# Distributed-Deep-Learning/MiniPs

Hardware: AMD Instinct MI355X
Metric: samples/sec (whole node) Criteo-shaped Wide&Deep BSP at 1/2/4/8 MI355X (higher is better)
Workload: dtype bf16; 1 GPU; global_batch=16384, parallelism=ps-dp1 (bsp; single rank: local shards, no collectives), per_gpu_batch=16384, consistency=bsp, world_size=1, backend=none, lookahead=2

## Files before the change

### csrc/kernels/widedeep.hip

```cpp
#include <cstdlib>
#include <stdexcept>
#include <string>
#include <utility>
#include <vector>

#include "common.h"
#include "kernels.h"

namespace minips_k {

__global__ void wd_assemble_kernel(const float* __restrict__ dense, int n_dense, const bf16_t* __restrict__ rows,
                                   int row_stride, const int64_t* __restrict__ inv, int64_t B, int F, int D,
                                   bf16_t* __restrict__ X, int ldx, float* __restrict__ wide_logit, int ones_col,
                                   float* __restrict__ zero_out) {
  if (zero_out && blockIdx.x == 0 && threadIdx.x == 0) *zero_out = 0.f;
  const int chunks = ldx >> 3;
  const int emb_cols = F * D;
  const int64_t total = B * chunks;
  const int64_t total_r = (total + 63) & ~63ll;
  for (int64_t c = blockIdx.x * (int64_t)blockDim.x + threadIdx.x; c < total_r + 32 * B;
       c += (int64_t)gridDim.x * blockDim.x) {
    if (c >= total_r) {
      const int64_t k = c - total_r, b = k >> 5;
      const int f = (int)(k & 31);
      float w = f < F ? bf2f(rows[inv[b * F + f] * row_stride + D]) : 0.f;
#pragma unroll
      for (int o = 16; o > 0; o >>= 1) w += __shfl_xor(w, o, 64);
      if (f == 0) wide_logit[b] = w;
      continue;
    }
    if (c >= total) continue;
    const int64_t b = c / chunks;
    const int col0 = (int)(c - b * chunks) * 8;
    uint32_t packed[4];
    if (col0 + 8 <= emb_cols && (D & 7) == 0) {
      const int f = col0 / D, d = col0 - f * D;
      const bf16_t* src = rows + inv[b * F + f] * row_stride + d;
      const uint2 lo = *reinterpret_cast<const uint2*>(src);
      const uint2 hi = *reinterpret_cast<const uint2*>(src + 4);
      packed[0] = lo.x;
      packed[1] = lo.y;
      packed[2] = hi.x;
      packed[3] = hi.y;
    } else {
      float v[8];
#pragma unroll
      for (int j = 0; j < 8; ++j) {
        const int col = col0 + j;
        if (col < emb_cols) {
          const int f = col / D, d = col - f * D;
          v[j] = bf2f(rows[inv[b * F + f] * row_stride + d]);
        } else if (col < emb_cols + n_dense) {
          v[j] = dense[b * n_dense + (col - emb_cols)];
        } else {
          v[j] = col == ones_col ? 1.f : 0.f;
        }
      }
#pragma unroll
      for (int j = 0; j < 4; ++j) packed[j] = pack_bf2(v[2 * j], v[2 * j + 1]);
    }
    *reinterpret_cast<uint4*>(X + b * ldx + col0) = make_uint4(packed[0], packed[1], packed[2], packed[3]);
  }
}

void wd_assemble(const float* dense, int n_dense, const bf16_t* rows, int row_stride, const int64_t* inv, int64_t B,
                 int F, int D, bf16_t* X, int ldx, float* wide_logit, int ones_col, hipStream_t s, float* zero_out) {
  if (ldx % 8) throw std::runtime_error("wd_assemble: ldx must be a multiple of 8");
  if (F * D + n_dense > ldx) throw std::runtime_error("wd_assemble: ldx too small");
  if (ones_col >= ldx) throw std::runtime_error("wd_assemble: ones_col out of range");
  if (row_stride % 4) throw std::runtime_error("wd_assemble: row_stride must be a multiple of 4");
  if (B <= 0) return;
  const int block = 256;
  if (F > 32) throw std::runtime_error("wd_assemble: at most 32 features");
  const int64_t items = ((B * (ldx / 8) + 63) & ~63ll) + 32 * B;
  hipLaunchKernelGGL(wd_assemble_kernel, (int)((items + block - 1) / block), block, 0, s, dense, n_dense, rows,
                     row_stride, inv, B, F, D, X, ldx, wide_logit, ones_col, zero_out);
  MINIPS_HIP_CHECK(hipGetLastError());
}

__global__ void wd_assemble_tab_kernel(const float* __restrict__ dense, int n_dense, const float* __restrict__ tab,
                                       int64_t tab_ld, const int64_t* __restrict__ uniq, int64_t base,
                                       const int64_t* __restrict__ inv, int64_t B, int F, int D,
                                       bf16_t* __restrict__ X, int ldx, float* __restrict__ wide_logit, int ones_col,
                                       float* __restrict__ zero_out, const int32_t* __restrict__ rowidx) {
  if (zero_out && blockIdx.x == 0 && threadIdx.x == 0) *zero_out = 0.f;
  const int chunks = ldx >> 3;
  const int emb_cols = F * D;
  const int64_t total = B * chunks;
  const int64_t total_r = (total + 63) & ~63ll;
  auto row_of = [&](int64_t b, int f) {
    const int64_t r = rowidx ? (int64_t)rowidx[b * F + f] : uniq[inv[b * F + f]];
    return tab + (r - base) * tab_ld;
  };
  for (int64_t c = blockIdx.x * (int64_t)blockDim.x + threadIdx.x; c < total_r + 32 * B;
       c += (int64_t)gridDim.x * blockDim.x) {
    if (c >= total_r) {
      const int64_t k = c - total_r, b = k >> 5;
      const int f = (int)(k & 31);
      float w = f < F ? __uint_as_float(pack_bf2(row_of(b, f)[D], 0.f) << 16) : 0.f;
#pragma unroll
      for (int o = 16; o > 0; o >>= 1) w += __shfl_xor(w, o, 64);
      if (f == 0) wide_logit[b] = w;
      continue;
    }
    if (c >= total) continue;
    const int64_t b = c / chunks;
    const int col0 = (int)(c - b * chunks) * 8;
    uint32_t packed[4];
    if (col0 + 8 <= emb_cols && (D & 7) == 0) {
      const int f = col0 / D, d = col0 - f * D;
      const float* src = row_of(b, f) + d;
      const float4 lo = *reinterpret_cast<const float4*>(src);
      const float4 hi = *reinterpret_cast<const float4*>(src + 4);
      packed[0] = pack_bf2(lo.x, lo.y);
      packed[1] = pack_bf2(lo.z, lo.w);
      packed[2] = pack_bf2(hi.x, hi.y);
      packed[3] = pack_bf2(hi.z, hi.w);
    } else {
      float v[8];
#pragma unroll
      for (int j = 0; j < 8; ++j) {
        const int col = col0 + j;
        if (col < emb_cols) {
          const int f = col / D, d = col - f * D;
          v[j] = __uint_as_float(pack_bf2(row_of(b, f)[d], 0.f) << 16);
        } else if (col < emb_cols + n_dense) {
          v[j] = dense[b * n_dense + (col - emb_cols)];
        } else {
          v[j] = col == ones_col ? 1.f : 0.f;
        }
      }
#pragma unroll
      for (int j = 0; j < 4; ++j) packed[j] = pack_bf2(v[2 * j], v[2 * j + 1]);
    }
    *reinterpret_cast<uint4*>(X + b * ldx + col0) = make_uint4(packed[0], packed[1], packed[2], packed[3]);
  }
}

void wd_assemble_tab(const float* dense, int n_dense, const float* tab, int64_t tab_ld, const int64_t* uniq,
                     int64_t base, const int64_t* inv, int64_t B, int F, int D, bf16_t* X, int ldx,
                     float* wide_logit, int ones_col, hipStream_t s, float* zero_out, const int32_t* rowidx) {
  if (ldx % 8) throw std::runtime_error("wd_assemble_tab: ldx must be a multiple of 8");
  if (F * D + n_dense > ldx) throw std::runtime_error("wd_assemble_tab: ldx too small");
  if (ones_col >= ldx) throw std::runtime_error("wd_assemble_tab: ones_col out of range");
  if (tab_ld % 4 || (D & 7) || tab_ld < D + 1) throw std::runtime_error("wd_assemble_tab: 16-byte rows, D % 8 == 0");
  if (F > 32) throw std::runtime_error("wd_assemble_tab: at most 32 features");
  if (B <= 0) return;
  const int block = 256;
  const int64_t items = ((B * (ldx / 8) + 63) & ~63ll) + 32 * B;
  hipLaunchKernelGGL(wd_assemble_tab_kernel, (int)((items + block - 1) / block), block, 0, s, dense, n_dense, tab,
                     tab_ld, uniq, base, inv, B, F, D, X, ldx, wide_logit, ones_col, zero_out, rowidx);
  MINIPS_HIP_CHECK(hipGetLastError());
// ... 519 lines not shown

__device__ __forceinline__ int block_excl_scan256(int v, int* sh, int* total) {
  const int lane = threadIdx.x & 63, w = threadIdx.x >> 6;
  int x = v;
#pragma unroll
  for (int o = 1; o < 64; o <<= 1) {
    const int y = __shfl_up(x, o, 64);
    if (lane >= o) x += y;
  }
  if (lane == 63) sh[w] = x;
  __syncthreads();
  int base = 0;
  for (int i = 0; i < w; ++i) base += sh[i];
  *total = sh[0] + sh[1] + sh[2] + sh[3];
  __syncthreads();
  return base + x - v;
}

__global__ __launch_bounds__(256) void emb_scan_reduce_kernel(const int* __restrict__ counts, int U,
                                                              int* __restrict__ tile_sums) {
  __shared__ int sh[4];
  const int i0 = blockIdx.x * kScanTile + threadIdx.x * 4;
  int v = 0;
#pragma unroll
  for (int q = 0; q < 4; ++q) v += (i0 + q < U) ? counts[i0 + q] : 0;
  int tot;
  block_excl_scan256(v, sh, &tot);
  if (threadIdx.x == 0) tile_sums[blockIdx.x] = tot;
}

__global__ __launch_bounds__(256) void emb_scan_top_kernel(int* __restrict__ tile_sums, int ntiles) {
  __shared__ int sh[4];
  int carry = 0;
  for (int base = 0; base < ntiles; base += 256) {
    const int i = base + threadIdx.x;
    const int v = i < ntiles ? tile_sums[i] : 0;
    int tot;
    const int ex = block_excl_scan256(v, sh, &tot);
    if (i < ntiles) tile_sums[i] = carry + ex;
    carry += tot;
  }
}

__global__ __launch_bounds__(256) void emb_scan_final_kernel(const int* __restrict__ counts, int U,
                                                             const int* __restrict__ tile_prefix,
                                                             int* __restrict__ offsets) {
  __shared__ int sh[4];
  const int i0 = blockIdx.x * kScanTile + threadIdx.x * 4;
  int c[4], v = 0;
#pragma unroll
  for (int q = 0; q < 4; ++q) {
    c[q] = (i0 + q < U) ? counts[i0 + q] : 0;
    v += c[q];
  }
  int tot;
  int run = tile_prefix[blockIdx.x] + block_excl_scan256(v, sh, &tot);
#pragma unroll
  for (int q = 0; q < 4; ++q) {
    if (i0 + q < U) offsets[i0 + q] = run;
    run += c[q];
  }
  if (blockIdx.x == gridDim.x - 1 && threadIdx.x == 255) offsets[U] = tile_prefix[blockIdx.x] + tot;
}

__global__ __launch_bounds__(kEmbTB) void emb_seg_fill_kernel(const int64_t* __restrict__ inv, int64_t B, int F,
                                                              const int* __restrict__ offsets,
                                                              int* __restrict__ cursor, int* __restrict__ members,
                                                              int* __restrict__ memrow) {
  __shared__ TileDedupe T;
  const int t = threadIdx.x, f = blockIdx.y;
  const int64_t b0 = (int64_t)blockIdx.x * kEmbTB;
  const int nb = (int)min((int64_t)kEmbTB, B - b0);
  int r, di, rank;
  tile_dedupe(T, inv, b0, nb, F, f, t, r, di, rank);
  if (t < T.nd) T.base[t] = offsets[T.rowof[t]] + atomicAdd(cursor + T.rowof[t], T.cnt[t]);
  __syncthreads();
  if (t < nb) {
    const int pos = T.base[di] + rank;
    members[pos] = (int)((b0 + t) * F + f);
    memrow[pos] = r;
  }
}

__device__ __forceinline__ float4 ld_grad4(const float* p) { return *reinterpret_cast<const float4*>(p); }
__device__ __forceinline__ float4 ld_grad4(const bf16_t* p) {
  const uint2 u = *reinterpret_cast<const uint2*>(p);
  return make_float4(__uint_as_float(u.x << 16), __uint_as_float(u.x & 0xffff0000u), __uint_as_float(u.y << 16),
                     __uint_as_float(u.y & 0xffff0000u));
}

template <int VW>
__device__ __forceinline__ void ld_gradv(const bf16_t* p, float (&v)[VW]) {
  if constexpr (VW == 8) {
    const uint4 u = *reinterpret_cast<const uint4*>(p);
    const uint32_t w[4] = {u.x, u.y, u.z, u.w};
#pragma unroll
    for (int e = 0; e < 4; ++e) {
      v[2 * e] = __uint_as_float(w[e] << 16);
      v[2 * e + 1] = __uint_as_float(w[e] & 0xffff0000u);
    }
  } else {
    const float4 f = ld_grad4(p);
    v[0] = f.x; v[1] = f.y; v[2] = f.z; v[3] = f.w;
  }
}
template <int VW>
__device__ __forceinline__ void ld_gradv(const float* p, float (&v)[VW]) {
#pragma unroll
  for (int h = 0; h < VW / 4; ++h) {
    const float4 f = *reinterpret_cast<const float4*>(p + 4 * h);
    v[4 * h] = f.x; v[4 * h + 1] = f.y; v[4 * h + 2] = f.z; v[4 * h + 3] = f.w;
  }
}

template <int VW>
__device__ __forceinline__ void st_row_vals(float* p, const float (&v)[VW]) {
#pragma unroll
  for (int h = 0; h < VW / 4; ++h)
    reinterpret_cast<float4*>(p)[h] = make_float4(v[4 * h], v[4 * h + 1], v[4 * h + 2], v[4 * h + 3]);
}
template <int VW>
__device__ __forceinline__ void st_row_vals(bf16_t* p, const float (&v)[VW]) {
#pragma unroll
  for (int h = 0; h < VW / 4; ++h)
    reinterpret_cast<uint2*>(p)[h] = make_uint2(pack_bf2(v[4 * h], v[4 * h + 1]), pack_bf2(v[4 * h + 2], v[4 * h + 3]));
}
__device__ __forceinline__ void st_scalar(float* p, float v) { *p = v; }
__device__ __forceinline__ void st_scalar(bf16_t* p, float v) { *p = f2bf(v); }

template <typename TO, int D, int VW>
__device__ __forceinline__ void seg_store_row(TO* __restrict__ out, int row_stride, int row, const float (&acc)[VW],
                                              float accw, bool wide, int l) {
  TO* o = out + (int64_t)row * row_stride;
  if ((row_stride & 3) == 0) {
    st_row_vals<VW>(o + VW * l, acc);
  } else {
#pragma unroll
    for (int e = 0; e < VW; ++e) st_scalar(o + VW * l + e, acc[e]);
  }
  if (l == 0)
    for (int c = D; c < row_stride; ++c) st_scalar(o + c, (c == D && wide) ? accw : 0.f);
}

constexpr int seg_part_stride(int D) { return D + 4; }

template <int D, int VW>
__device__ __forceinline__ void seg_store_part(float* __restrict__ part, int64_t slot, const float (&acc)[VW],
                                               float accw, int l) {
  float* o = part + slot * seg_part_stride(D);
  st_row_vals<VW>(o + VW * l, acc);
  if (l == 0) o[D] = accw;
}

template <typename TX, typename TO, int D, int G, int BATCH, bool SORTED, int VW>
__global__ __launch_bounds__(256) void emb_seg_det_kernel(const TX* __restrict__ dX, int ldx,
                                                          const float* __restrict__ dwide, int F,
                                                          const int* __restrict__ members,
                                                          const int* __restrict__ memrow, int total,
                                                          TO* __restrict__ out, int row_stride,
                                                          float* __restrict__ part) {
  constexpr int L = D / VW, PER = 64 / L, PW = PER * G;
  const int lane = threadIdx.x & 63, sub = lane / L, l = lane % L;
  const bool wide = dwide != nullptr;
  const int64_t wave = (blockIdx.x * (int64_t)blockDim.x + threadIdx.x) >> 6;
  const int64_t nw = ((int64_t)gridDim.x * blockDim.x) >> 6;
  for (int64_t piece = wave; piece * PW < total; piece += nw) {
    const int wbase = (int)(piece * PW);
    const int a = wbase + sub * G, b = min(total, a + G);
    const bool has = a < b;
    const int prev_row = (has && a > 0) ? memrow[a - 1] : -1;
    const int next_row = (has && b < total) ? memrow[b] : -1;
    const int wave_prev = wbase > 0 ? memrow[wbase - 1] : -1;
    int cur = -1, rf = -1, rl = -1;
    bool first = true, hasF = false, interior = false, hasL = false;
    float acc[VW], fv[VW], lv[VW];
#pragma unroll
    for (int e = 0; e < VW; ++e) acc[e] = fv[e] = lv[e] = 0.f;
    float accw = 0.f, fw = 0.f, lw = 0.f;
    for (int m0 = a; m0 < b; m0 += BATCH) {
      int u[BATCH], bb[BATCH];
      float v[BATCH][VW];
      float vw[BATCH];
#pragma unroll
      for (int q = 0; q < BATCH; ++q) {
        const int m = m0 + q;
        u[q] = m < b ? memrow[m] : -1;
        const TX* src;
        if (SORTED) {
          src = dX + (int64_t)(m < b ? m : a) * D + VW * l;
          bb[q] = (wide && l == 0 && m < b) ? members[m] / F : 0;
        } else {
          const int j = m < b ? members[m] : members[a];
          bb[q] = j / F;
          const int ff = j - bb[q] * F;
          src = dX + (int64_t)bb[q] * ldx + ff * D + VW * l;
        }
        ld_gradv<VW>(src, v[q]);
        vw[q] = (wide && l == 0 && m < b) ? dwide[bb[q]] : 0.f;
      }
#pragma unroll
      for (int q = 0; q < BATCH; ++q) {
        if (u[q] < 0) break;
        if (u[q] != cur) {
          if (cur >= 0) {
            if (first && cur == prev_row) {
#pragma unroll
              for (int e = 0; e < VW; ++e) fv[e] = acc[e];
              fw = accw;
              hasF = true;
              rf = cur;
            } else {
              seg_store_row<TO, D, VW>(out, row_stride, cur, acc, accw, wide, l);
            }
            first = false;
          }
          cur = u[q];
#pragma unroll
          for (int e = 0; e < VW; ++e) acc[e] = 0.f;
          accw = 0.f;
        }
#pragma unroll
        for (int e = 0; e < VW; ++e) acc[e] += v[q][e];
        accw += vw[q];
      }
    }
    if (cur >= 0) {
      if (first && cur == prev_row) {
#pragma unroll
        for (int e = 0; e < VW; ++e) fv[e] = acc[e];
        fw = accw;
        hasF = true;
        rf = cur;
        interior = cur == next_row;
      } else if (cur == next_row) {
#pragma unroll
        for (int e = 0; e < VW; ++e) lv[e] = acc[e];
        lw = accw;
        hasL = true;
        rl = cur;
      } else {
        seg_store_row<TO, D, VW>(out, row_stride, cur, acc, accw, wide, l);
      }
    }
    float cv[VW];
#pragma unroll
    for (int e = 0; e < VW; ++e) cv[e] = 0.f;
    float cw = 0.f;
    int crow = -1;
    const int src = (lane - L) & 63;
#pragma unroll
    for (int s = 0; s < PER; ++s) {
      float iv[VW];
#pragma unroll
      for (int e = 0; e < VW; ++e) iv[e] = __shfl(cv[e], src, 64);
      const float iw = __shfl(cw, src, 64);
      const int irow = __shfl(crow, src, 64);
      if (sub == s) {
        const bool carried = s > 0 && irow >= 0 && irow == rf;
        if (hasF) {
          float tv[VW];
#pragma unroll
          for (int e = 0; e < VW; ++e) tv[e] = carried ? iv[e] + fv[e] : fv[e];
          const float tw = carried ? iw + fw : fw;
          if (interior) {
#pragma unroll
            for (int e = 0; e < VW; ++e) cv[e] = tv[e];
            cw = tw;
            crow = rf;
          } else {
            if (wbase > 0 && rf == wave_prev) seg_store_part<D, VW>(part, 2 * piece, tv, tw, l);
            else seg_store_row<TO, D, VW>(out, row_stride, rf, tv, tw, wide, l);
#pragma unroll
            for (int e = 0; e < VW; ++e) cv[e] = lv[e];
            cw = lw;
            crow = hasL ? rl : -1;
          }
        } else {
#pragma unroll
          for (int e = 0; e < VW; ++e) cv[e] = lv[e];
          cw = lw;
          crow = hasL ? rl : -1;
        }
      }
    }
    if (sub == PER - 1 && crow >= 0) seg_store_part<D, VW>(part, 2 * piece + 1, cv, cw, l);
  }
}

template <typename TO, int D, int VW, int PW>
__global__ __launch_bounds__(256) void emb_seg_fix_kernel(const int* __restrict__ memrow, int total,
                                                          const float* __restrict__ part, TO* __restrict__ out,
                                                          int row_stride, bool wide) {
  constexpr int L = D / VW, PER = 64 / L, SP = seg_part_stride(D);
  const int lane = threadIdx.x & 63, sub = lane / L, l = lane % L;
  const int64_t npieces = ((int64_t)total + PW - 1) / PW;
  const int64_t wave = (blockIdx.x * (int64_t)blockDim.x + threadIdx.x) >> 6;
  const int64_t nw = ((int64_t)gridDim.x * blockDim.x) >> 6;
  for (int64_t p = wave; p < npieces; p += nw) {
    const int bw = (int)(p * PW), ew = (int)min((int64_t)total, (p + 1) * PW);
    const int r = memrow[ew - 1];
    if (!(ew < total && memrow[ew] == r)) continue;
    if (bw > 0 && memrow[bw] == r && memrow[bw - 1] == r) continue;
    float s[VW];
#pragma unroll
    for (int e = 0; e < VW; ++e) s[e] = 0.f;
    float sw = 0.f;
    constexpr int QPG = 4;
    for (int64_t w0 = p;; w0 += PER * QPG) {
      bool end = false;
#pragma unroll
      for (int k = 0; k < QPG; ++k) {
      const int64_t q = w0 + k * PER + sub;
      const bool valid = q < npieces;
      const int64_t qc = valid ? q : p;
      const int mb = memrow[qc * PW];
      const int64_t eq = min((int64_t)total, (qc + 1) * PW);
      const int me = eq < total ? memrow[eq] : -1;
      const float* ph = part + (2 * qc) * SP;
      const float* pt = ph + SP;
      float vh[VW], vt[VW];
      ld_gradv<VW>(ph + VW * l, vh);
      ld_gradv<VW>(pt + VW * l, vt);
      const float wh = ph[D], wt = pt[D];
      const bool in = valid && (q == p || mb == r);
      const bool through = in && me == r;
      const bool tail = q == p || through;
      if (in) {
#pragma unroll
        for (int e = 0; e < VW; ++e) s[e] += tail ? vt[e] : vh[e];
        sw += tail ? wt : wh;
      }
      end = end || !through;
      }
      if (__any(end)) break;
    }
#pragma unroll
    for (int o = L; o < 64; o <<= 1) {
#pragma unroll
      for (int e = 0; e < VW; ++e) s[e] += __shfl_xor(s[e], o, 64);
      sw += __shfl_xor(sw, o, 64);
    }
    if (sub == 0) seg_store_row<TO, D, VW>(out, row_stride, r, s, sw, wide, l);
  }
}

void emb_build_csr(const int64_t* inv, int64_t B, int F, int U, int* ws, int* members, int* memrow, hipStream_t s,
                   int* zeroed_cc, bool counts_ready) {
  if (B <= 0 || U <= 0) return;
  int* counts = zeroed_cc ? zeroed_cc : ws;
  int* cursor = counts + U;
  int* offsets = zeroed_cc ? ws : cursor + U;
  int* tiles = offsets + U + 1;
  const int ntiles = (U + kScanTile - 1) / kScanTile;
  if (!zeroed_cc) MINIPS_HIP_CHECK(hipMemsetAsync(counts, 0, sizeof(int) * 2 * (size_t)U, s));
  dim3 grid((unsigned)((B + kEmbTB - 1) / kEmbTB), (unsigned)F);
  if (!(counts_ready && zeroed_cc)) hipLaunchKernelGGL(emb_seg_count_kernel, grid, dim3(kEmbTB), 0, s, inv, B,
                                                       F, counts);
  hipLaunchKernelGGL(emb_scan_reduce_kernel, ntiles, 256, 0, s, counts, U, tiles);
  hipLaunchKernelGGL(emb_scan_top_kernel, 1, 256, 0, s, tiles, ntiles);
  hipLaunchKernelGGL(emb_scan_final_kernel, ntiles, 256, 0, s, counts, U, tiles, offsets);
  hipLaunchKernelGGL(emb_seg_fill_kernel, grid, dim3(kEmbTB), 0, s, inv, B, F, offsets, cursor, members, memrow);
  MINIPS_HIP_CHECK(hipGetLastError());
}

constexpr int kSegG = 16, kSegBatch = 8, kSegVW = 4;

constexpr int seg_per_piece(int D) { return (64 / (D / kSegVW)) * kSegG; }

int64_t emb_seg_part_floats(int64_t total, int D) {
  const int64_t pw = seg_per_piece(D);
  return 2 * ((total + pw - 1) / pw) * seg_part_stride(D);
}

template <typename TX, typename TO>
static void emb_seg_det(const TX* dX, int ldx, const float* dwide, int64_t B, int F, int D, const int* members,
                        const int* memrow, TO* out, int row_stride, float* part, hipStream_t s, bool sorted_rows) {
  const int total = (int)(B * F);
  const int64_t pw = seg_per_piece(D);
  const int64_t pieces = (total + pw - 1) / pw;
  const int blocks = (int)std::max<int64_t>(1, std::min<int64_t>((pieces + 3) / 4, 65535));
  const int fix_blocks = (int)std::max<int64_t>(1, std::min<int64_t>((pieces + 3) / 4, 4096));
#define MINIPS_SEG_DET(DD)                                                                                         \
  if (sorted_rows)                                                                                                \
    hipLaunchKernelGGL((emb_seg_det_kernel<TX, TO, DD, kSegG, kSegBatch, true, kSegVW>), blocks, 256, 0, s, dX,    \
                       ldx, dwide, F, members, memrow, total, out, row_stride, part);                             \
  else                                                                                                            \
    hipLaunchKernelGGL((emb_seg_det_kernel<TX, TO, DD, kSegG, kSegBatch, false, kSegVW>), blocks, 256, 0, s, dX,   \
                       ldx, dwide, F, members, memrow, total, out, row_stride, part);                             \
  if (pieces > 1)                                                                                                 \
    hipLaunchKernelGGL((emb_seg_fix_kernel<TO, DD, kSegVW, seg_per_piece(DD)>), fix_blocks, 256, 0, s, memrow,     \
                       total, part, out, row_stride, dwide != nullptr);
  switch (D) {
    case 16:
      MINIPS_SEG_DET(16)
      break;
    case 32:
      MINIPS_SEG_DET(32)
      break;
    case 64:
      MINIPS_SEG_DET(64)
      break;
    default:
      throw std::runtime_error("emb_backward_seg: D must be 16, 32 or 64");
  }
#undef MINIPS_SEG_DET
  MINIPS_HIP_CHECK(hipGetLastError());
}

void emb_backward_csr(const void* dX, bool bf16, int ldx, const float* dwide, int64_t B, int F, int D,
                      const int* members, const int* memrow, void* out, bool out_bf16, int row_stride, float* part,
                      hipStream_t s, bool sorted_rows) {
  if (B <= 0) return;
  if (row_stride < D + (dwide ? 1 : 0)) throw std::runtime_error("emb_backward_csr: row_stride too small");
  if (bf16 && out_bf16)
    emb_seg_det(static_cast<const bf16_t*>(dX), ldx, dwide, B, F, D, members, memrow, static_cast<bf16_t*>(out),
                row_stride, part, s, sorted_rows);
  else if (bf16)
    emb_seg_det(static_cast<const bf16_t*>(dX), ldx, dwide, B, F, D, members, memrow, static_cast<float*>(out),
                row_stride, part, s, sorted_rows);
  else if (out_bf16)
    emb_seg_det(static_cast<const float*>(dX), ldx, dwide, B, F, D, members, memrow, static_cast<bf16_t*>(out),
                row_stride, part, s, sorted_rows);
  else
    emb_seg_det(static_cast<const float*>(dX), ldx, dwide, B, F, D, members, memrow, static_cast<float*>(out),
                row_stride, part, s, sorted_rows);
}

__global__ void emb_csr_positions_kernel(const int* __restrict__ members, int64_t n, int* __restrict__ pos) {
  for (int64_t m = blockIdx.x * (int64_t)blockDim.x + threadIdx.x; m < n; m += (int64_t)gridDim.x * blockDim.x)
    pos[members[m]] = (int)m;
}

void emb_csr_positions(const int* members, int64_t n, int* pos, hipStream_t s) {
  if (n <= 0) return;
  hipLaunchKernelGGL(emb_csr_positions_kernel, grid_for(n, 256, 4096), 256, 0, s, members, n, pos);
  MINIPS_HIP_CHECK(hipGetLastError());
}

void emb_backward_segment(const void* dX, bool bf16, int ldx, const float* dwide, const int64_t* inv, int64_t B, int F,
                          int D, void* out, bool out_bf16, int row_stride, int U, int* ws, float* part, hipStream_t s) {
  if (B <= 0 || U <= 0) return;
  int* members = ws + 3 * U + 1 + (U / 1024 + 1);
  int* memrow = members + B * F;
  emb_build_csr(inv, B, F, U, ws, members, memrow, s);
  emb_backward_csr(dX, bf16, ldx, dwide, B, F, D, members, memrow, out, out_bf16, row_stride, part, s, false);
}

}
```

### minips_amd/ops/__init__.py

```python
from __future__ import annotations

import math

import torch

from .._native import evalk, ftrlk, kernels, optk, wdftrlk

EPI_STORE_F32 = 0
EPI_ATOMIC_F32 = 1
EPI_BIAS_RELU_BF16 = 2
EPI_BIAS_BF16 = 3
EPI_STORE_BF16 = 4
EPI_RELU_MASK_BF16 = 5
EPI_BIAS_GELU_BF16 = 6
EPI_BIAS_GELU_AUX_BF16 = 7
EPI_GELU_GRAD_BF16 = 8
EPI_PERM_ROWS_BF16 = 9
EPI_BIAS_GELU_DAUX_BF16 = 13
EPI_MUL_AUX_BF16 = 14
_L2E = 1.4426950408889634


def _gelu_grad(u):
    k, c = 0.7978845608, 0.044715
# ... 475 lines not shown
        out = torch.empty(B, rows.shape[1], dtype=torch.float32, device=rows.device)
    if _gpu(rows):
        kernels().embedding_bag_fwd(rows, idx, offsets, bool(mean), out)
        return out
    mode = "mean" if mean else "sum"
    out.copy_(torch.nn.functional.embedding_bag(idx, rows, offsets[:-1], mode=mode, include_last_offset=False))
    return out


def embedding_bag_bwd(grad_out, idx, offsets, grad_rows, mean=False):
    if _gpu(grad_out):
        kernels().embedding_bag_bwd(grad_out, idx, offsets, bool(mean), grad_rows)
        return grad_rows
    lens = (offsets[1:] - offsets[:-1])
    bag = torch.repeat_interleave(torch.arange(lens.numel(), device=idx.device), lens)
    g = grad_out[bag]
    if mean:
        g = g / lens[bag].clamp_min(1).unsqueeze(1).to(g.dtype)
    grad_rows.index_add_(0, idx, g)
    return grad_rows


def wd_assemble(dense, rows, inv, F, D, X, wide_logit, ones_col=-1, zero=None):
    if _gpu(X):
        kernels().wd_assemble(dense, rows, inv, int(F), int(D), X, wide_logit, int(ones_col), zero)
        return X, wide_logit
    if zero is not None:
        zero.zero_()
    B = X.shape[0]
    r = rows[inv].view(B, F, rows.shape[1]).float()
    X.zero_()
    X[:, : F * D] = r[:, :, :D].reshape(B, F * D).to(torch.bfloat16)
    X[:, F * D: F * D + dense.shape[1]] = dense.to(torch.bfloat16)
    if ones_col >= 0:
        X[:, ones_col] = 1.0
    wide_logit.copy_(r[:, :, D].sum(1))
    return X, wide_logit


def wd_assemble_tab(dense, table, index, base, inv, F, D, X, wide_logit, ones_col=-1, zero=None, rowidx=None):
    if _gpu(X):
        kernels().wd_assemble_tab(dense, table, index, int(base), inv, int(F), int(D), X, wide_logit, int(ones_col),
                                  zero, rowidx)
        return X, wide_logit
    U = int(inv.max()) + 1 if inv.numel() else 0
    rows = table[index[:U] - base].to(torch.bfloat16)
    return wd_assemble(dense, rows, inv, F, D, X, wide_logit, ones_col, zero)


def wd_head(H, w, b0, wide_logit, labels, dH, dw, db, dwide, loss_sum, dH_colsum=None, grad_scale=1.0,
            defer_fold=False):
    if _gpu(H):
        kernels().wd_head(H, w, b0, wide_logit, labels, dH, dw, db, dwide, loss_sum, dH_colsum, float(grad_scale),
                          bool(defer_fold))
        return
    h = H.float()
    z = h @ w.float() + b0.float() + wide_logit
    y = (labels > 0.5).float()
    p = torch.sigmoid(z)
    dz = (p - y) * grad_scale
    dwide.copy_(dz)
    db += dz.sum()
    loss_sum += (torch.clamp_min(z, 0) - z * y + torch.log1p(torch.exp(-z.abs()))).sum()
    g = torch.where(h > 0, dz.unsqueeze(1) * w.float().unsqueeze(0), torch.zeros_like(h)).to(torch.bfloat16)
    dH.copy_(g)
    dw += (dz.unsqueeze(1) * h).sum(0)
    if dH_colsum is not None:
        dH_colsum += g.float().sum(0)


def wd_head_fold(B, Hd, dw, db, loss_sum, dH_colsum=None):
    if _gpu(dw):
        (kernels() if _REC is None else _REC.lst).wd_head_fold(int(B), int(Hd), dw, db, loss_sum, dH_colsum)


EVAL_LOSS_SCALE = float(1 << 24)


def _eval_bins(acc) -> int:
    NB = (acc.numel() - 2) // 2
    if acc.dtype != torch.int64 or acc.numel() != 2 * NB + 2 or not 32 <= NB <= 8192 or NB & (NB - 1):
        raise RuntimeError(f"acc must be int64 [2*NB + 2] with NB a power of two in [32, 8192], got "
                           f"{acc.dtype} [{acc.numel()}]")
    return NB


def binary_hist(logits, labels, acc):
    NB = _eval_bins(acc)
    if _gpu(logits):
        evalk().binary_hist(logits, labels, acc)
        return
    z = logits.reshape(-1).to(torch.float32)
    y = labels.reshape(-1).to(torch.float32) > 0.5
    ok = ~torch.isnan(z)
    acc[2 * NB + 1] += int((~ok).sum())
    z, y = z[ok], y[ok]
    zc = torch.clamp(z, -16.0, 16.0)
    bins = torch.clamp_max(torch.floor((zc + 16.0) * float(NB // 32)).to(torch.int64), NB - 1)
    acc[:NB] += torch.bincount(bins[~y], minlength=NB)
    acc[NB:2 * NB] += torch.bincount(bins[y], minlength=NB)
    zl = torch.clamp(z, -64.0, 64.0)
    l = torch.clamp_min(zl, 0) - zl * y.to(torch.float32) + torch.log1p(torch.exp(-zl.abs()))
    acc[2 * NB] += torch.round(l * EVAL_LOSS_SCALE).to(torch.int64).sum()


def eval_head(H, w, b0, wide, labels, acc, logits_out=None):
    if _gpu(H):
        evalk().eval_head_hist(H, w, b0, wide, labels, acc, logits_out)
        return
    z = H.float() @ w.float() + b0.float()
    if wide is not None:
        z = z + wide
    if logits_out is not None:
        logits_out.copy_(z)
    binary_hist(z, labels, acc)


def emb_csr_positions(members):
    if _gpu(members):
        return kernels().emb_csr_positions(members)
    pos = torch.empty_like(members)
    pos[members.long()] = torch.arange(members.numel(), dtype=members.dtype)
    return pos


def emb_build_csr(inv, F, U, zeroed=None, counts_ready=False):
    if _gpu(inv):
        return tuple(kernels().emb_build_csr(inv, int(F), int(max(U, 1)), zeroed, bool(counts_ready)))
    order = torch.sort(inv, stable=True).indices
    return order.to(torch.int32), inv[order].to(torch.int32)


def wd_emb_backward(dX, dwide, inv, F, D, grad_rows, x_off=0, csr=None, sorted_rows=False):
    if _gpu(dX):
        members, memrow = (csr[0], csr[1]) if csr is not None else (None, None)
        kernels().wd_emb_backward(dX, dwide, inv, int(F), int(D), grad_rows, int(x_off), members, memrow,
                                  bool(sorted_rows))
        return grad_rows
    if sorted_rows:
        un = torch.empty_like(dX)
        un[csr[0].long()] = dX
        dX, x_off = un.reshape(-1, F * D), 0
    B = dX.shape[0]
    g = dX[:, x_off: x_off + F * D].float().reshape(B * F, D)
    acc = grad_rows if grad_rows.dtype == torch.float32 else grad_rows.float()
    acc[:, :D].index_add_(0, inv, g)
    if dwide is not None:
        acc[:, D].index_add_(0, inv, dwide.repeat_interleave(F))
    if acc is not grad_rows:
        grad_rows.copy_(acc)
    return grad_rows


def _slab_args(slabs):
    return [(s, int(n), int(p), int(o)) for s, n, p, o in slabs]


def _fold_slabs(g, slabs, group4=True):
    if not slabs:
        return g
    x = g.clone()
    for s, n, p, o in slabs:
        P, r = s[: n * p].view(n, p), x[o: o + p]
        z = 0
        while group4 and z + 3 < n:
            r += (P[z] + P[z + 1]) + (P[z + 2] + P[z + 3])
            z += 4
        while z < n:
            r += P[z]
            z += 1
    return x


def adam_apply(w, m, v, g, lr, beta1=0.9, beta2=0.999, eps=1e-8, weight_decay=0.0, step=1, grad_scale=1.0,
               w_bf16=None, step_dev=None, zero_g=False, slabs=()):
    if _gpu(w):
        kernels().adam_apply(w, m, v, g, float(lr), float(beta1), float(beta2), float(eps), float(weight_decay),
                             int(step), float(grad_scale), w_bf16, step_dev, bool(zero_g), _slab_args(slabs))
        return
    g_in, g = g, _fold_slabs(g, slabs)
    if step_dev is not None:
        step = int(step_dev.reshape(-1)[0])
    gg = g * grad_scale
    m.mul_(beta1).add_((1 - beta1) * gg)
    v.mul_(beta2).add_((1 - beta2) * gg * gg)
    bc1, bc2 = 1 - beta1 ** step, 1 - beta2 ** step
    w.sub_(lr * ((m / bc1) / ((v / bc2).sqrt() + eps) + weight_decay * w))
    if w_bf16 is not None:
        w_bf16.copy_(w.to(torch.bfloat16))
    if zero_g:
        g_in.zero_()


def grad_sumsq(g, part, L=None, slabs=()):
    L = part.numel() if L is None else int(L)
    if _gpu(g):
        optk().grad_sumsq(g, _slab_args(slabs), part, L)
        return part
    if not 1 <= L <= 1024 or part.numel() < L or part.dtype != torch.float64:
        raise RuntimeError(f"grad_sumsq: part must be float64 with 1 <= L <= 1024 entries, got {part.dtype} "
                           f"[{part.numel()}], L {L}")
    part[:L] = 0
    part[0] = _fold_slabs(g, slabs).double().square().sum()
    return part


def clip_scale(total: float, max_norm: float):
    if not math.isfinite(total):
        return math.sqrt(total) if total > 0 else float("nan"), 0.0, True
    norm = math.sqrt(total)
    sd = max_norm / (norm + 1e-6)
    return norm, (float(torch.tensor(sd, dtype=torch.float32)) if sd < 1.0 else 1.0), False


def adam_clip_apply(w, m, v, g, lr, part, max_norm, stats, beta1=0.9, beta2=0.999, eps=1e-8, weight_decay=0.0,
                    step=1, np=None, w_bf16=None, step_dev=None, zero_g=False, slabs=(), write_stats=True):
    np = part.numel() if np is None else int(np)
    if _gpu(w):
        optk().adam_clip_apply(w, m, v, g, _slab_args(slabs), float(lr), float(beta1), float(beta2), float(eps),
                               float(weight_decay), int(step), step_dev, w_bf16, bool(zero_g), part, np,
                               float(max_norm), stats, bool(write_stats))
        return
    if not 1 <= np <= 4096 or part.numel() < np:
        raise RuntimeError(f"adam_clip_apply: np {np} outside [1, 4096] or beyond part [{part.numel()}]")
    norm, scale, skip = clip_scale(float(part[:np].sum()), float(max_norm))
    if write_stats:
        stats[0], stats[1] = norm, scale
        stats[3 if skip else 2] += 1.0 if skip or scale < 1.0 else 0.0
    if not skip:
        adam_apply(w, m, v, _fold_slabs(g, slabs), lr, beta1, beta2, eps, weight_decay, step, scale, w_bf16,
                   step_dev=step_dev)
    if zero_g:
        g.zero_()


def slab_pack(g, out, slabs=()):
    if _gpu(g):
        kernels().slab_pack(g, out, _slab_args(slabs))
        return out
    out.copy_(_fold_slabs(g, slabs, group4=False))
    g.zero_()
    return out


def sgd_apply(w, g, lr, grad_scale=1.0, w_bf16=None):
    if _gpu(w):
        kernels().sgd_apply(w, g, float(lr), float(grad_scale), w_bf16)
        return
    w.sub_(lr * grad_scale * g)
    if w_bf16 is not None:
        w_bf16.copy_(w.to(torch.bfloat16))


def adagrad_apply(w, acc, g, lr, eps=1e-10, grad_scale=1.0, w_bf16=None):
    if _gpu(w):
        kernels().adagrad_apply(w, acc, g, float(lr), float(eps), float(grad_scale), w_bf16)
        return
    gg = g * grad_scale
    acc.add_(gg * gg)
    w.sub_(lr * gg / (acc.sqrt() + eps))
    if w_bf16 is not None:
        w_bf16.copy_(w.to(torch.bfloat16))


def cast_f32_bf16(x, y):
    if _gpu(x):
        kernels().cast_f32_bf16(x, y)
        return y
    y.copy_(x.to(torch.bfloat16))
    return y


def lr_sparse_step(rowptr, cols, vals, labels, w, alpha, delta=None, correct=None):
    if _gpu(w):
        kernels().lr_sparse_step(rowptr, cols, vals, labels, w, float(alpha), delta, correct)
        return
    B = labels.numel()
    lens = rowptr[1:] - rowptr[:-1]
    row = torch.repeat_interleave(torch.arange(B, device=w.device), lens)
    dot = torch.zeros(B, dtype=w.dtype, device=w.device).index_add_(0, row, w[cols] * vals)
    p = torch.sigmoid(dot)
    y = labels.clamp_min(0)
    err = alpha * (y - p)
    if delta is not None:
        delta.index_add_(0, cols, err[row] * vals)
    if correct is not None:
        correct += ((p > 0.5) == (y > 0.5)).float().sum()


def kmeans_assign_csr(rowptr, cols, vals, C, assign=None, dist=None):
    n = rowptr.numel() - 1
    if assign is None:
        assign = torch.empty(n, dtype=torch.int32, device=C.device)
    if _gpu(C):
        cnorm = torch.empty(C.shape[0], dtype=torch.float32, device=C.device)
        kernels().kmeans_assign_csr(rowptr, cols, vals, C, cnorm, assign, dist)
        return assign
    lens = rowptr[1:] - rowptr[:-1]
    row = torch.repeat_interleave(torch.arange(n, device=C.device), lens)
    ok = cols < C.shape[1]
    xn = torch.zeros(n, dtype=torch.float32).index_add_(0, row, vals * vals)
    dots = torch.zeros(n, C.shape[0], dtype=torch.float32)
    dots.index_add_(0, row[ok], vals[ok, None] * C[:, cols[ok]].t())
    d2 = xn[:, None] - 2 * dots + (C * C).sum(1)[None]
    best, idx = d2.min(1)
    assign.copy_(idx.to(torch.int32))
# ... 301 lines not shown
```

Measured before the change: 49.03 million samples/s.

## Restructure segmented embedding backward with prefetched keys, lane-shared indices and magic division

The deterministic segmented-sum embedding backward kernel now loads each group's member/row keys cooperatively, spreading them across lanes and broadcasting them with shuffles. It prefetches the next piece's keys while the current piece accumulates, replaces integer division by F with a magic-multiply that is self-checked on the host, and uses 32-bit offsets when the data fits. The fix kernel runs one wave per block and double-buffers its partial loads. Launch uses 64-thread blocks with a capped grid that can be overridden by an environment variable. The aim is to cut memory latency and integer-op overhead in the gradient scatter, at the cost of more register pressure and more code complexity.

```diff
diff --git a/csrc/kernels/widedeep.hip b/csrc/kernels/widedeep.hip
--- a/csrc/kernels/widedeep.hip
+++ b/csrc/kernels/widedeep.hip
@@ -1,3 +1,4 @@
+#include <atomic>
 #include <cstdlib>
 #include <stdexcept>
 #include <string>
@@ -823,80 +824,156 @@
   if (l == 0) o[D] = accw;
 }
 
-template <typename TX, typename TO, int D, int G, int BATCH, bool SORTED, int VW>
+struct SegDiv {
+  uint32_t mul;
+  int shift;
+};
+static SegDiv seg_div_magic(int F) {
+  int s = 0;
+  while ((1ll << s) < F) ++s;
+  return SegDiv{(uint32_t)((((uint64_t)1 << (31 + s)) + (uint64_t)F - 1) / (uint64_t)F), s};
+}
+__host__ __device__ __forceinline__ int seg_div(int j, SegDiv d) {
+#if defined(__HIP_DEVICE_COMPILE__)
+  return (int)(__umulhi((uint32_t)j << 1, d.mul) >> d.shift);
+#else
+  return (int)((uint32_t)((((uint64_t)(uint32_t)j << 1) * d.mul) >> 32) >> d.shift);
+#endif
+}
+
+struct SegRawBf { uint2 u; };
+struct SegRawF { float4 f; };
+__device__ __forceinline__ SegRawBf seg_ld_raw(const bf16_t* p) { return SegRawBf{*reinterpret_cast<const uint2*>(p)}; }
+__device__ __forceinline__ SegRawF seg_ld_raw(const float* p) { return SegRawF{*reinterpret_cast<const float4*>(p)}; }
+__device__ __forceinline__ SegRawBf seg_pad_raw(const SegRawBf& r, bool valid) {
+  return SegRawBf{make_uint2(valid ? r.u.x : 0x80008000u, valid ? r.u.y : 0x80008000u)};
+}
+__device__ __forceinline__ SegRawF seg_pad_raw(const SegRawF& r, bool valid) {
+  return SegRawF{make_float4(valid ? r.f.x : -0.f, valid ? r.f.y : -0.f, valid ? r.f.z : -0.f, valid ? r.f.w : -0.f)};
+}
+__device__ __forceinline__ void seg_add_raw(float (&acc)[4], const SegRawBf& r) {
+  acc[0] += __uint_as_float(r.u.x << 16);
+  acc[1] += __uint_as_float(r.u.x & 0xffff0000u);
+  acc[2] += __uint_as_float(r.u.y << 16);
+  acc[3] += __uint_as_float(r.u.y & 0xffff0000u);
+}
+__device__ __forceinline__ void seg_add_raw(float (&acc)[4], const SegRawF& r) {
+  acc[0] += r.f.x; acc[1] += r.f.y; acc[2] += r.f.z; acc[3] += r.f.w;
+}
+
+template <typename TO, int D, int VW>
+__device__ __forceinline__ void seg_flush_row(TO* __restrict__ out, int row_stride, int row, const float (&acc)[VW],
+                                              float accw, bool wide, int l) {
+  if (row_stride == D + 4) {
+    TO* o = out + (int64_t)row * (D + 4);
+    st_row_vals<VW>(o + VW * l, acc);
+    if (l == 0) {
+      const float t[4] = {wide ? accw : 0.f, 0.f, 0.f, 0.f};
+      st_row_vals<4>(o + D, t);
+    }
+  } else {
+    seg_store_row<TO, D, VW>(out, row_stride, row, acc, accw, wide, l);
+  }
+}
+
+template <typename TX, typename TO, int D, int G, bool SORTED, int VW, typename OffT>
 __global__ __launch_bounds__(256) void emb_seg_det_kernel(const TX* __restrict__ dX, int ldx,
-                                                          const float* __restrict__ dwide, int F,
-                                                          const int* __restrict__ members,
-                                                          const int* __restrict__ memrow, int total,
-                                                          TO* __restrict__ out, int row_stride,
-                                                          float* __restrict__ part) {
-  constexpr int L = D / VW, PER = 64 / L, PW = PER * G;
-  const int lane = threadIdx.x & 63, sub = lane / L, l = lane % L;
+                                                         const float* __restrict__ dwide, int F, SegDiv fdiv,
+                                                         const int* __restrict__ members,
+                                                         const int* __restrict__ memrow, int total,
+                                                         TO* __restrict__ out, int row_stride,
+                                                         float* __restrict__ part) {
+  static_assert(VW == 4 && G % (D / VW) == 0, "a lane holds 4 values and a whole share of its group's entries");
+  constexpr int L = D / VW, PER = 64 / L, PW = PER * G, E = G / L;
+  const int lane = threadIdx.x & 63, sub = lane / L, l = lane % L, gbase = lane - l;
+  const int wv = __builtin_amdgcn_readfirstlane(threadIdx.x >> 6), wpb = blockDim.x >> 6;
   const bool wide = dwide != nullptr;
-  const int64_t wave = (blockIdx.x * (int64_t)blockDim.x + threadIdx.x) >> 6;
-  const int64_t nw = ((int64_t)gridDim.x * blockDim.x) >> 6;
-  for (int64_t piece = wave; piece * PW < total; piece += nw) {
+  struct Keys {
+    int mu[E], mj[E], wp, wn;
+  };
+  auto load_keys = [&](int64_t pc, Keys& k) {
+    const int wb = (int)(pc * PW);
+    const int ka = (int)min((int64_t)wb + sub * G, (int64_t)total);
+#pragma unroll
+    for (int e = 0; e < E; ++e) {
+      const int idx = ka + min(l * E + e, total - 1 - ka);
+      k.mu[e] = memrow[idx];
+      k.mj[e] = (!SORTED || wide) ? members[idx] : 0;
+    }
+    k.wp = memrow[max(wb - 1, 0)];
+    k.wn = memrow[(int)min((int64_t)wb + PW, (int64_t)total - 1)];
+  };
+  const int64_t npieces = ((int64_t)total + PW - 1) / PW, stride = (int64_t)gridDim.x * wpb;
+  int64_t piece = (int64_t)blockIdx.x * wpb + wv;
+  if (piece >= npieces) return;
+  const float* wsrc = wide ? dwide : reinterpret_cast<const float*>(memrow);
+  const uint32_t wmask = wide ? 0xffffffffu : 0u;
+  Keys kc;
+  load_keys(piece, kc);
+  for (;;) {
     const int wbase = (int)(piece * PW);
-    const int a = wbase + sub * G, b = min(total, a + G);
-    const bool has = a < b;
-    const int prev_row = (has && a > 0) ? memrow[a - 1] : -1;
-    const int next_row = (has && b < total) ? memrow[b] : -1;
-    const int wave_prev = wbase > 0 ? memrow[wbase - 1] : -1;
-    int cur = -1, rf = -1, rl = -1;
-    bool first = true, hasF = false, interior = false, hasL = false;
+    const int a = (int)min((int64_t)wbase + sub * G, (int64_t)total);
+    const int cnt = min(G, total - a);
+    int mu[E], mj[E];
+#pragma unroll
+    for (int e = 0; e < E; ++e) mu[e] = kc.mu[e], mj[e] = kc.mj[e];
+    const int wp = kc.wp, wn = kc.wn;
+    const int wave_prev = wbase > 0 ? wp : -1;
+    const int wave_next = (int64_t)wbase + PW < total ? wn : -1;
+    OffT mo[E];
+    float mw[E];
+#pragma unroll
+    for (int e = 0; e < E; ++e) {
+      const int bb = seg_div(mj[e], fdiv);
+      if (SORTED) mo[e] = (OffT)(a + min(l * E + e, total - 1 - a)) * D;
+      else mo[e] = (OffT)bb * ldx + (mj[e] - bb * F) * D;
+      mw[e] = __uint_as_float(__float_as_uint(wsrc[bb & wmask]) & wmask);
+    }
+    int u[G];
+    decltype(seg_ld_raw(dX)) raw[G];
+#pragma unroll
+    for (int q = 0; q < G; ++q) {
+      u[q] = __shfl(mu[q % E], gbase + q / E, 64);
+      const OffT off = __shfl(mo[q % E], gbase + q / E, 64);
+      raw[q] = seg_ld_raw(dX + off + VW * l);
+    }
+    const int64_t nxt = piece + stride;
+    if (nxt < npieces) load_keys(nxt, kc);
+    const int up = __shfl(mu[E - 1], (gbase - 1) & 63, 64), un = __shfl(mu[0], (gbase + L) & 63, 64);
+    const int prev_row = a > 0 ? (sub > 0 ? up : wave_prev) : -1;
+    const int next_row = (int64_t)a + G < total ? (sub < PER - 1 ? un : wave_next) : -1;
+    float vw[G];
+#pragma unroll
+    for (int q = 0; q < G; ++q) vw[q] = __shfl(mw[q % E], gbase + q / E, 64);
+    int rf = -1, rl = -1;
+    bool pendF = cnt > 0 && u[0] == prev_row, hasF = false, interior = false, hasL = false;
     float acc[VW], fv[VW], lv[VW];
 #pragma unroll
     for (int e = 0; e < VW; ++e) acc[e] = fv[e] = lv[e] = 0.f;
     float accw = 0.f, fw = 0.f, lw = 0.f;
-    for (int m0 = a; m0 < b; m0 += BATCH) {
-      int u[BATCH], bb[BATCH];
-      float v[BATCH][VW];
-      float vw[BATCH];
-#pragma unroll
-      for (int q = 0; q < BATCH; ++q) {
-        const int m = m0 + q;
-        u[q] = m < b ? memrow[m] : -1;
-        const TX* src;
-        if (SORTED) {
-          src = dX + (int64_t)(m < b ? m : a) * D + VW * l;
-          bb[q] = (wide && l == 0 && m < b) ? members[m] / F : 0;
+#pragma unroll
+    for (int q = 0; q < G; ++q) {
+      if (q > 0 && u[q] != u[q - 1]) {
+        if (pendF) {
+#pragma unroll
+          for (int e = 0; e < VW; ++e) fv[e] = acc[e];
+          fw = accw;
+          hasF = true;
+          rf = u[q - 1];
+          pendF = false;
         } else {
-          const int j = m < b ? members[m] : members[a];
-          bb[q] = j / F;
-          const int ff = j - bb[q] * F;
-          src = dX + (int64_t)bb[q] * ldx + ff * D + VW * l;
+          seg_flush_row<TO, D, VW>(out, row_stride, u[q - 1], acc, accw, wide, l);
         }
-        ld_gradv<VW>(src, v[q]);
-        vw[q] = (wide && l == 0 && m < b) ? dwide[bb[q]] : 0.f;
+#pragma unroll
+        for (int e = 0; e < VW; ++e) acc[e] = 0.f;
+        accw = 0.f;
       }
-#pragma unroll
-      for (int q = 0; q < BATCH; ++q) {
-        if (u[q] < 0) break;
-        if (u[q] != cur) {
-          if (cur >= 0) {
-            if (first && cur == prev_row) {
-#pragma unroll
-              for (int e = 0; e < VW; ++e) fv[e] = acc[e];
-              fw = accw;
-              hasF = true;
-              rf = cur;
-            } else {
-              seg_store_row<TO, D, VW>(out, row_stride, cur, acc, accw, wide, l);
-            }
-            first = false;
-          }
-          cur = u[q];
-#pragma unroll
-          for (int e = 0; e < VW; ++e) acc[e] = 0.f;
-          accw = 0.f;
-        }
-#pragma unroll
-        for (int e = 0; e < VW; ++e) acc[e] += v[q][e];
-        accw += vw[q];
-      }
-    }
-    if (cur >= 0) {
-      if (first && cur == prev_row) {
+      seg_add_raw(acc, seg_pad_raw(raw[q], q < cnt));
+      accw += q < cnt ? vw[q] : -0.f;
+    }
+    if (cnt > 0) {
+      const int cur = u[G - 1];
+      if (pendF) {
 #pragma unroll
         for (int e = 0; e < VW; ++e) fv[e] = acc[e];
         fw = accw;
@@ -910,7 +987,7 @@
         hasL = true;
         rl = cur;
       } else {
-        seg_store_row<TO, D, VW>(out, row_stride, cur, acc, accw, wide, l);
+        seg_flush_row<TO, D, VW>(out, row_stride, cur, acc, accw, wide, l);
       }
     }
     float cv[VW];
@@ -940,7 +1017,7 @@
             crow = rf;
           } else {
             if (wbase > 0 && rf == wave_prev) seg_store_part<D, VW>(part, 2 * piece, tv, tw, l);
-            else seg_store_row<TO, D, VW>(out, row_stride, rf, tv, tw, wide, l);
+            else seg_flush_row<TO, D, VW>(out, row_stride, rf, tv, tw, wide, l);
 #pragma unroll
             for (int e = 0; e < VW; ++e) cv[e] = lv[e];
             cw = lw;
@@ -955,55 +1032,75 @@
       }
     }
     if (sub == PER - 1 && crow >= 0) seg_store_part<D, VW>(part, 2 * piece + 1, cv, cw, l);
-  }
-}
+    if (nxt >= npieces) break;
+    piece = nxt;
+  }
+}
+
+template <int D, int VW, int PW, int QPG>
+struct SegFixWindow {
+  int mb[QPG], me[QPG];
+  float vh[QPG][VW], vt[QPG][VW], wh[QPG], wt[QPG];
+  __device__ __forceinline__ void load(const int* __restrict__ memrow, int total, const float* __restrict__ part,
+                                       int64_t npieces, int64_t p, int64_t w0, int sub, int l) {
+    constexpr int PER = 64 / (D / VW), SP = seg_part_stride(D);
+#pragma unroll
+    for (int k = 0; k < QPG; ++k) {
+      const int64_t q = w0 + k * PER + sub;
+      const int64_t qc = q < npieces ? q : p;
+      mb[k] = memrow[qc * PW];
+      const int64_t eq = min((int64_t)total, (qc + 1) * PW);
+      const int mk = memrow[min(eq, (int64_t)total - 1)];
+      me[k] = eq < total ? mk : -1;
+      const float* ph = part + (2 * qc) * SP;
+      const float* pt = ph + SP;
+      ld_gradv<VW>(ph + VW * l, vh[k]);
+      ld_gradv<VW>(pt + VW * l, vt[k]);
+      wh[k] = ph[D];
+      wt[k] = pt[D];
+    }
+  }
+};
 
 template <typename TO, int D, int VW, int PW>
-__global__ __launch_bounds__(256) void emb_seg_fix_kernel(const int* __restrict__ memrow, int total,
-                                                          const float* __restrict__ part, TO* __restrict__ out,
-                                                          int row_stride, bool wide) {
-  constexpr int L = D / VW, PER = 64 / L, SP = seg_part_stride(D);
-  const int lane = threadIdx.x & 63, sub = lane / L, l = lane % L;
+__global__ __launch_bounds__(64) void emb_seg_fix_kernel(const int* __restrict__ memrow, int total,
+                                                         const float* __restrict__ part, TO* __restrict__ out,
+                                                         int row_stride, bool wide) {
+  constexpr int L = D / VW, PER = 64 / L;
+  constexpr int QPG = 4;
+  const int lane = threadIdx.x, sub = lane / L, l = lane % L;
   const int64_t npieces = ((int64_t)total + PW - 1) / PW;
-  const int64_t wave = (blockIdx.x * (int64_t)blockDim.x + threadIdx.x) >> 6;
-  const int64_t nw = ((int64_t)gridDim.x * blockDim.x) >> 6;
-  for (int64_t p = wave; p < npieces; p += nw) {
+  for (int64_t p = blockIdx.x; p < npieces; p += gridDim.x) {
     const int bw = (int)(p * PW), ew = (int)min((int64_t)total, (p + 1) * PW);
     const int r = memrow[ew - 1];
-    if (!(ew < total && memrow[ew] == r)) continue;
-    if (bw > 0 && memrow[bw] == r && memrow[bw - 1] == r) continue;
+    const int rnl = memrow[min(ew, total - 1)], rbl = memrow[max(bw - 1, 0)];
+    const int rn = ew < total ? rnl : -1;
+    const int rb = memrow[bw], rbp = bw > 0 ? rbl : -1;
+    SegFixWindow<D, VW, PW, QPG> w;
+    w.load(memrow, total, part, npieces, p, p, sub, l);
+    const bool active = (rn == r) & !((bw > 0) & (rb == r) & (rbp == r));
     float s[VW];
 #pragma unroll
     for (int e = 0; e < VW; ++e) s[e] = 0.f;
     float sw = 0.f;
-    constexpr int QPG = 4;
-    for (int64_t w0 = p;; w0 += PER * QPG) {
+    for (int64_t w0 = p;;) {
       bool end = false;
 #pragma unroll
       for (int k = 0; k < QPG; ++k) {
-      const int64_t q = w0 + k * PER + sub;
-      const bool valid = q < npieces;
-      const int64_t qc = valid ? q : p;
-      const int mb = memrow[qc * PW];
-      const int64_t eq = min((int64_t)total, (qc + 1) * PW);
-      const int me = eq < total ? memrow[eq] : -1;
-      const float* ph = part + (2 * qc) * SP;
-      const float* pt = ph + SP;
-      float vh[VW], vt[VW];
-      ld_gradv<VW>(ph + VW * l, vh);
-      ld_gradv<VW>(pt + VW * l, vt);
-      const float wh = ph[D], wt = pt[D];
-      const bool in = valid && (q == p || mb == r);
-      const bool through = in && me == r;
-      const bool tail = q == p || through;
-      if (in) {
-#pragma unroll
-        for (int e = 0; e < VW; ++e) s[e] += tail ? vt[e] : vh[e];
-        sw += tail ? wt : wh;
+        const int64_t q = w0 + k * PER + sub;
+        const bool in = q < npieces && (q == p || w.mb[k] == r);
+        const bool through = in && w.me[k] == r;
+        const bool tail = q == p || through;
+        if (in) {
+#pragma unroll
+          for (int e = 0; e < VW; ++e) s[e] += tail ? w.vt[k][e] : w.vh[k][e];
+          sw += tail ? w.wt[k] : w.wh[k];
+        }
+        end = end || !through;
       }
-      end = end || !through;
-      }
-      if (__any(end)) break;
+      if (__any(end) || !active) break;
+      w0 += PER * QPG;
+      w.load(memrow, total, part, npieces, p, w0, sub, l);
     }
 #pragma unroll
     for (int o = L; o < 64; o <<= 1) {
@@ -1011,9 +1108,10 @@
       for (int e = 0; e < VW; ++e) s[e] += __shfl_xor(s[e], o, 64);
       sw += __shfl_xor(sw, o, 64);
     }
-    if (sub == 0) seg_store_row<TO, D, VW>(out, row_stride, r, s, sw, wide, l);
-  }
-}
+    if (sub == 0 && active) seg_flush_row<TO, D, VW>(out, row_stride, r, s, sw, wide, l);
+  }
+}
+
 
 void emb_build_csr(const int64_t* inv, int64_t B, int F, int U, int* ws, int* members, int* memrow, hipStream_t s,
                    int* zeroed_cc, bool counts_ready) {
@@ -1034,13 +1132,25 @@
   MINIPS_HIP_CHECK(hipGetLastError());
 }
 
-constexpr int kSegG = 16, kSegBatch = 8, kSegVW = 4;
+constexpr int kSegG = 16, kSegVW = 4;
 
 constexpr int seg_per_piece(int D) { return (64 / (D / kSegVW)) * kSegG; }
 
 int64_t emb_seg_part_floats(int64_t total, int D) {
   const int64_t pw = seg_per_piece(D);
   return 2 * ((total + pw - 1) / pw) * seg_part_stride(D);
+}
+
+static void seg_div_selfcheck(int F, SegDiv d) {
+  static std::atomic<bool> checked[65];
+  if (F <= 64 && checked[F].load(std::memory_order_relaxed)) return;
+  const int64_t lim = (int64_t)1 << 31;
+  for (int64_t base : {(int64_t)0, (int64_t)1 << 20, lim - 1 - 2 * (int64_t)F}) {
+    const int64_t m0 = base / F * F;
+    for (int64_t j = std::max<int64_t>(0, m0 - 2); j <= m0 + 2 * F + 1 && j < lim; ++j)
+      if (seg_div((int)j, d) != (int)(j / F)) throw std::runtime_error("emb_backward_seg: inexact lookup-id division");
+  }
+  if (F <= 64) checked[F].store(true, std::memory_order_relaxed);
 }
 
 template <typename TX, typename TO>
@@ -1049,18 +1159,29 @@
   const int total = (int)(B * F);
   const int64_t pw = seg_per_piece(D);
   const int64_t pieces = (total + pw - 1) / pw;
-  const int blocks = (int)std::max<int64_t>(1, std::min<int64_t>((pieces + 3) / 4, 65535));
-  const int fix_blocks = (int)std::max<int64_t>(1, std::min<int64_t>((pieces + 3) / 4, 4096));
+  const int blocks = (int)std::max<int64_t>(1, std::min<int64_t>(pieces, 1 << 20));
+  constexpr int tpb = 64;
+  static const int gcap = getenv("MINIPS_SEG_GRID") ? atoi(getenv("MINIPS_SEG_GRID")) : 832;
+  int dblocks = (int)((pieces + tpb / 64 - 1) / (tpb / 64));
+  if (gcap > 0) dblocks = std::min(dblocks, gcap);
+  dblocks = std::max(1, std::min(dblocks, 1 << 20));
+  const SegDiv fdiv = seg_div_magic(F);
+  seg_div_selfcheck(F, fdiv);
+  const bool idx32 = (sorted_rows ? (int64_t)total * D : B * (int64_t)ldx) * (int64_t)sizeof(TX) < ((int64_t)1 << 31);
+#define MINIPS_SEG_DET_K(DD, SORTED, OFFT)                                                                         \
+  hipLaunchKernelGGL((emb_seg_det_kernel<TX, TO, DD, kSegG, SORTED, kSegVW, OFFT>), dblocks, tpb, 0, s, dX, ldx,    \
+                     dwide, F, fdiv, members, memrow, total, out, row_stride, part)
 #define MINIPS_SEG_DET(DD)                                                                                         \
-  if (sorted_rows)                                                                                                \
-    hipLaunchKernelGGL((emb_seg_det_kernel<TX, TO, DD, kSegG, kSegBatch, true, kSegVW>), blocks, 256, 0, s, dX,    \
-                       ldx, dwide, F, members, memrow, total, out, row_stride, part);                             \
-  else                                                                                                            \
-    hipLaunchKernelGGL((emb_seg_det_kernel<TX, TO, DD, kSegG, kSegBatch, false, kSegVW>), blocks, 256, 0, s, dX,   \
-                       ldx, dwide, F, members, memrow, total, out, row_stride, part);                             \
+  if (sorted_rows) {                                                                                              \
+    if (idx32) MINIPS_SEG_DET_K(DD, true, int);                                                                    \
+    else MINIPS_SEG_DET_K(DD, true, int64_t);                                                                      \
+  } else {                                                                                                        \
+    if (idx32) MINIPS_SEG_DET_K(DD, false, int);                                                                   \
+    else MINIPS_SEG_DET_K(DD, false, int64_t);                                                                     \
+  }                                                                                                               \
   if (pieces > 1)                                                                                                 \
-    hipLaunchKernelGGL((emb_seg_fix_kernel<TO, DD, kSegVW, seg_per_piece(DD)>), fix_blocks, 256, 0, s, memrow,     \
-                       total, part, out, row_stride, dwide != nullptr);
+    hipLaunchKernelGGL((emb_seg_fix_kernel<TO, DD, kSegVW, seg_per_piece(DD)>), blocks, 64, 0, s, memrow, total,   \
+                       part, out, row_stride, dwide != nullptr);
   switch (D) {
     case 16:
       MINIPS_SEG_DET(16)
@@ -1074,6 +1195,7 @@
     default:
       throw std::runtime_error("emb_backward_seg: D must be 16, 32 or 64");
   }
+#undef MINIPS_SEG_DET_K
 #undef MINIPS_SEG_DET
   MINIPS_HIP_CHECK(hipGetLastError());
 }
diff --git a/minips_amd/ops/__init__.py b/minips_amd/ops/__init__.py
--- a/minips_amd/ops/__init__.py
+++ b/minips_amd/ops/__init__.py
@@ -651,6 +651,127 @@
     return grad_rows
 
 
+_SEG_G = 16
+
+
+def _seg_per_piece(D):
+    return (64 // (D // 4)) * _SEG_G
+
+
+def _seg_div_magic(F):
+    s = 0
+    while (1 << s) < F:
+        s += 1
+    return ((1 << (31 + s)) + F - 1) // F, s
+
+
+def _seg_div(j, F):
+    mul, s = _seg_div_magic(F)
+    return (((2 * j) & 0xFFFFFFFF) * mul >> 32) >> s
+
+
+def _emb_seg_order_ref(dX, dwide, csr, F, D, grad_rows, x_off=0, sorted_rows=False):
+    import numpy as np
+
+    members, memrow = csr[0].numpy().astype(np.int64), csr[1].numpy().astype(np.int64)
+    total, G = len(members), _SEG_G
+    PER, PW = 64 // (D // 4), _seg_per_piece(D)
+    if sorted_rows:
+        X = dX.float().numpy().reshape(total, D)
+    else:
+        B = dX.shape[0]
+        X = dX[:, x_off: x_off + F * D].float().numpy().reshape(B * F, D)[members]
+    V = np.zeros((total, D + 1), np.float32)
+    V[:, :D] = X
+    wide = dwide is not None
+    if wide:
+        V[:, D] = dwide.float().numpy()[members // F]
+    W = grad_rows.shape[1]
+    res = grad_rows.float().numpy().copy()
+    zero = np.zeros(D + 1, np.float32)
+
+    def store(row, v):
+        res[row, :D] = v[:D]
+        if W > D:
+            res[row, D] = v[D] if wide else 0.0
+            res[row, D + 1:] = 0.0
+
+    npieces = (total + PW - 1) // PW
+    head, tail = np.zeros((npieces, D + 1), np.float32), np.zeros((npieces, D + 1), np.float32)
+    for p in range(npieces):
+        wbase = p * PW
+        wave_prev = memrow[wbase - 1] if wbase > 0 else -1
+        cv, crow = zero, -1
+        for s in range(PER):
+            a, b = wbase + s * G, min(total, wbase + (s + 1) * G)
+            fv = lv = zero
+            rf = rl = -1
+            hasF = interior = hasL = False
+            if a < b:
+                prev_row = memrow[a - 1] if a > 0 else -1
+                next_row = memrow[b] if b < total else -1
+                pendF = memrow[a] == prev_row
+                acc = zero.copy()
+                for m in range(a, b):
+                    if m > a and memrow[m] != memrow[m - 1]:
+                        if pendF:
+                            fv, rf, hasF, pendF = acc, memrow[m - 1], True, False
+                        else:
+                            store(memrow[m - 1], acc)
+                        acc = zero.copy()
+                    acc = acc + V[m]
+                cur = memrow[b - 1]
+                if pendF:
+                    fv, rf, hasF, interior = acc, cur, True, cur == next_row
+                elif cur == next_row:
+                    lv, rl, hasL = acc, cur, True
+                else:
+                    store(cur, acc)
+            if hasF:
+                tv = cv + fv if (s > 0 and crow >= 0 and crow == rf) else fv
+                if interior:
+                    cv, crow = tv, rf
+                    continue
+                if wbase > 0 and rf == wave_prev:
+                    head[p] = tv
+                else:
+                    store(rf, tv)
+            cv, crow = lv, (rl if hasL else -1)
+        if crow >= 0:
+            tail[p] = cv
+    QPG = 4
+    for p in range(npieces if npieces > 1 else 0):
+        bw, ew = p * PW, min(total, (p + 1) * PW)
+        r = memrow[ew - 1]
+        if not (ew < total and memrow[ew] == r):
+            continue
+        if bw > 0 and memrow[bw] == r and memrow[bw - 1] == r:
+            continue
+        sums = [zero.copy() for _ in range(PER)]
+        w0 = p
+        while True:
+            end = False
+            for g in range(PER):
+                for k in range(QPG):
+                    q = w0 + k * PER + g
+                    inside = q < npieces and (q == p or memrow[q * PW] == r)
+                    eq = min(total, (q + 1) * PW)
+                    through = inside and eq < total and memrow[eq] == r
+                    if inside:
+                        sums[g] = sums[g] + (tail[q] if (q == p or through) else head[q])
+                    end = end or not through
+            if end:
+                break
+            w0 += PER * QPG
+        o = 1
+        while o < PER:
+            sums = [sums[g] + sums[g ^ o] for g in range(PER)]
+            o *= 2
+        store(r, sums[0])
+    grad_rows.copy_(torch.from_numpy(res).to(grad_rows.dtype))
+    return grad_rows
+
+
 def _slab_args(slabs):
     return [(s, int(n), int(p), int(o)) for s, n, p, o in slabs]
 
```

Result: no change. 48.96 million samples/s (-0.2%).
